# ercembu/bulletproof-perm

Measured on NVIDIA B200. Metric: shuffle proofs/sec prove+verify (52-card), higher is better.
Workload: dtype u32 (8x32-bit limbs, IMAD.WIDE.U32)

## Files before the change

bulletproof-perm_b200/csrc/acproof_kernels.cuh:

```cuda
#pragma once
#include "ge25519.cuh"
#include "vec_kernels.cuh"

struct acp_layout {
    uint32_t n, Q, m, stride;
    uint32_t np, lg;
    uint32_t aL, aR, aO, gamma;
    uint32_t alpha, beta, ro, sl, sr, tau;
    uint32_t y, z, x, w;
    uint32_t yn, yninv, zq;
    uint32_t zWL, zWR, zWO, zWV, zc;
    uint32_t lin, l1, r0, r1, r3;
    uint32_t dots;
    uint32_t tc, tsel, sigma;
    uint32_t l, r, that, taux, mu;
    uint32_t vg, vh, vG, vH, vd;
    uint32_t rho, rho0;
    uint32_t wq, u, uinv, cl, pa, pb, ptab;
    uint32_t stab;
};

#define ACP_PTR(base, lay, p, off) ((base) + 8 * ((size_t)(p) * (lay).stride + (off)))

SC_INLINE uint32_t rotl32(uint32_t v, int n) { return (v << n) | (v >> (32 - n)); }
#define CHACHA_QR(a, b, c, d) \
    a += b; d = rotl32(d ^ a, 16); c += d; b = rotl32(b ^ c, 12); a += b; d = rotl32(d ^ a, 8); c += d; b = rotl32(b ^ c, 7);

__global__ void k_acp_rng(const uint32_t *__restrict__ seeds , acp_layout lay, uint32_t count,
                          uint32_t *__restrict__ blk) {
    const uint32_t j = blockIdx.x * blockDim.x + threadIdx.x, p = blockIdx.y;
    if (j >= count) return;
    uint32_t s[16], x[16];
    s[0] = 0x61707865u; s[1] = 0x3320646eu; s[2] = 0x79622d32u; s[3] = 0x6b206574u;
#pragma unroll
// ... 18 lines not shown
__global__ void __launch_bounds__(128) k_acp_place_witness(const uint32_t *__restrict__ st, acp_layout lay, uint32_t B,
                                                           uint32_t *__restrict__ blk) {
    const uint32_t i = blockIdx.x * blockDim.x + threadIdx.x, p = blockIdx.y;
    const uint32_t n = lay.n, m = lay.m;
    if (i >= 3 * n + m) return;
    const uint32_t which = i < 3 * n ? i / n : 3, k = i - which * n;
    const uint32_t *src = which < 3 ? st + 8 * (((size_t)which * B + p) * n + k) : st + 8 * ((size_t)3 * B * n + (size_t)p * m + k);
    const uint32_t off = which == 0 ? lay.aL : which == 1 ? lay.aR : which == 2 ? lay.aO : lay.gamma;
    uint4 lo = *reinterpret_cast<const uint4 *>(src), hi = *reinterpret_cast<const uint4 *>(src + 4);
    uint32_t *dst = ACP_PTR(blk, lay, p, off + k);
    *reinterpret_cast<uint4 *>(dst) = lo;
    *reinterpret_cast<uint4 *>(dst + 4) = hi;
}

#define WIT_THREADS 256
__global__ void __launch_bounds__(WIT_THREADS) k_shuffle_witness(const uint32_t *__restrict__ deck ,
                                                                 const uint32_t *__restrict__ perm ,
                                                                 const uint32_t *__restrict__ xs , uint32_t k,
                                                                 acp_layout lay, uint32_t *__restrict__ blk,
                                                                 uint32_t *__restrict__ vout ) {
    __shared__ __align__(16) uint32_t sh[2][WIT_THREADS * 8];
    const uint32_t c = blockIdx.x, p = blockIdx.y, tid = threadIdx.x;
    const uint32_t gb = c * (k - 1), vb = c * k, len = k - 1;
    const uint32_t T = blockDim.x;
    const uint32_t run = (len + T - 1) / T, i0 = tid * run, i1 = min(len, i0 + run);
    const uint32_t *pp = perm + (size_t)p * k;
    uint32_t *vp = vout + 8 * (size_t)p * lay.m;
    sc x, one, r2;
    sc_load(x, xs + 8 * (size_t)p);
    sc_const(one, SC_R);
    sc_const(r2, SC_R2);
    auto value = [&](uint32_t j) {
        sc v;
        BPP_ASSERT(j < k && (!c || pp[j] < k));
        sc_load(v, deck + 8 * (size_t)(c ? pp[j] : j));
        sc_store(vp + 8 * (size_t)(vb + j), v);
        return v;
    };
    sc acc = one, f, t;
    for (uint32_t i = i0; i < i1; i++) {
        f = value(i + 1);
        sc_sub(f, f, x);
        sc_store(ACP_PTR(blk, lay, p, lay.aR + gb + i), f);
        sc_mont(t, f, r2);
        sc_mont(acc, acc, t);
    }
    if (tid == 0) {
        f = value(0);
        sc_sub(f, f, x);
        sc_store(ACP_PTR(blk, lay, p, lay.aL + gb), f);
        sc_mont(t, f, r2);
        sc_mont(acc, acc, t);
        if (c == 0) {
            sc_store(vp + 8 * (size_t)(2 * k), x);
            sc z;
            sc_set0(z);
            for (uint32_t q = 2 * k - 2; q < 2 * k; q++) {
                sc_store(ACP_PTR(blk, lay, p, lay.aL + q), z);
                sc_store(ACP_PTR(blk, lay, p, lay.aR + q), z);
                sc_store(ACP_PTR(blk, lay, p, lay.aO + q), z);
            }
        }
    }
    int cur = 0;
    sc_store(sh[0] + 8 * tid, acc);
    __syncthreads();
    for (uint32_t d = 1; d < T; d <<= 1) {
        sc a, b2;
        sc_load(a, sh[cur] + 8 * tid);
// ... 33 lines not shown
    const uint32_t *pp = perm + (size_t)p * k;
    uint32_t *vp = vout + 8 * (size_t)p * lay.m;
    sc x, r2, v, f, fm, P;
    sc_load(x, xs + 8 * (size_t)p);
    sc_const(r2, SC_R2);
    BPP_ASSERT(!c || pp[0] < k);
    sc_load(v, deck + 8 * (size_t)(c ? pp[0] : 0));
    sc_store(vp + 8 * (size_t)vb, v);
    sc_sub(P, v, x);
    sc_store(ACP_PTR(blk, lay, p, lay.aL + gb), P);
#pragma unroll 1
    for (uint32_t i = 0; i < len; i++) {
        BPP_ASSERT(!c || pp[i + 1] < k);
        sc_load(v, deck + 8 * (size_t)(c ? pp[i + 1] : i + 1));
        sc_store(vp + 8 * (size_t)(vb + i + 1), v);
        sc_sub(f, v, x);
        sc_store(ACP_PTR(blk, lay, p, lay.aR + gb + i), f);
        if (i) sc_store(ACP_PTR(blk, lay, p, lay.aL + gb + i), P);
        sc_mont_noinline(fm, f, r2);
        sc_mont_noinline(P, P, fm);
        sc_store(ACP_PTR(blk, lay, p, lay.aO + gb + i), P);
    }
    if (c == 0) {
        sc_store(vp + 8 * (size_t)(2 * k), x);
        sc z;
        sc_set0(z);
        for (uint32_t q = 2 * k - 2; q < 2 * k; q++) {
            sc_store(ACP_PTR(blk, lay, p, lay.aL + q), z);
            sc_store(ACP_PTR(blk, lay, p, lay.aR + q), z);
            sc_store(ACP_PTR(blk, lay, p, lay.aO + q), z);
        }
    }
}
__global__ void __launch_bounds__(128) k_acp_place_gamma(const uint32_t *__restrict__ st, acp_layout lay, uint32_t *__restrict__ blk) {
    const uint32_t i = blockIdx.x * blockDim.x + threadIdx.x, p = blockIdx.y;
    if (i >= lay.m) return;
    const uint32_t *src = st + 8 * ((size_t)p * lay.m + i);
    uint4 lo = *reinterpret_cast<const uint4 *>(src), hi = *reinterpret_cast<const uint4 *>(src + 4);
    uint32_t *dst = ACP_PTR(blk, lay, p, lay.gamma + i);
// ... 40 lines not shown
        ge_affine_to_niels(e, x, y);
        ge_niels_store(dst + FB_ENTRY_U32 * (size_t)(j - 1), e);
        if (j < half) ge_add_noinline(run, run, base);
    }
}

struct fb_shape {
    uint32_t nseg;
    uint32_t sc_off[4];
    uint32_t sc_ostride[4];
    uint32_t gen[4];
    uint32_t cnt[4];
    uint32_t outs;
    uint32_t sel_period;
    uint32_t sel[4];
};
struct fb_consts {
    uint32_t K[8];
};
#ifndef FB_THREADS
#define FB_THREADS 128
#endif
#ifndef FB_GROUP
#define FB_GROUP 4
#endif

static __host__ __device__ __forceinline__ uint32_t fb_terms(const fb_shape &sh) {
    uint32_t n = 0;
    for (uint32_t s = 0; s < sh.nseg; s++) n += sh.cnt[s];
    return n;
// ... 159 lines not shown
            *reinterpret_cast<uint4 *>(stage + 8 * (size_t)t + 4) = hi;
        }
        __syncwarp();
    }
    uint32_t s[9];
    ge_ext acc;
    fb_accumulate_items(acc, s, sh, table, c, Wn, kc, o, total_terms, lane, 32, [&](uint32_t seg, uint32_t k, uint32_t term) {
        return STAGE ? stage + 8 * (size_t)term : fb_scalar(blk, lay, sh, p, o, seg, k);
    });
    ge_warp_sum<false>(acc);
    if (lane == 0) ge_store(out_ext + 32 * ((size_t)p * sh.outs + o), acc);
}
#ifndef FB_STAGE_MAX_BYTES
#define FB_STAGE_MAX_BYTES (48u * 1024u)
#endif
template <int C>
__global__ void __launch_bounds__(FB_THREADS, FB_WARP_MINBLOCKS) k_fb_msm_warp_d(const uint32_t *__restrict__ blk, acp_layout lay, fb_shape sh,
                                                              const uint32_t *__restrict__ table, fb_consts kc,
                                                              uint32_t B, uint32_t outs ,
                                                              uint32_t *__restrict__ out_ext ) {
    constexpr uint32_t WN = (256 + C - 1) / C, LOG_WN = WN == 32 ? 5 : 4, HALF = 1u << (C - 1);
    static_assert((C == 16 && WN == 16) || (C == 8 && WN == 32), "window count must be a power of two dividing 32");
    extern __shared__ __align__(16) uint32_t fb_stage[];
    const uint32_t wid = blockIdx.x * (FB_THREADS / 32) + (threadIdx.x >> 5), lane = threadIdx.x & 31;
    if (wid >= B * outs) return;
    const uint32_t p = wid / outs, o = wid - p * outs;
    const uint32_t total_terms = fb_terms(sh);
    uint32_t *stage = fb_stage + (size_t)(threadIdx.x >> 5) * ((9 * total_terms + 3) & ~3u);
    uint32_t *sgen = stage + 8 * (size_t)total_terms;
    uint32_t n_act = 0;
    for (uint32_t t0 = 0; t0 < total_terms; t0 += 32) {
        const uint32_t t = t0 + lane;
        bool act = t < total_terms;
        uint32_t seg = 0, k = t;
        if (act) {
            fb_locate_term(sh, t, seg, k);
            act = fb_term_selected(sh, seg, k, o);
        }
        const uint32_t bal = __ballot_sync(0xffffffffu, act);
        if (act) {
            const uint32_t idx = n_act + __popc(bal & ((1u << lane) - 1u));
            uint32_t s[8];
            const uint32_t carry = fb_recode(fb_scalar(blk, lay, sh, p, o, seg, k), kc.K, s);
            BPP_ASSERT(carry == 0 && idx < total_terms);
            (void)carry;
            *reinterpret_cast<uint4 *>(stage + 8 * (size_t)idx) = make_uint4(s[0], s[1], s[2], s[3]);
            *reinterpret_cast<uint4 *>(stage + 8 * (size_t)idx + 4) = make_uint4(s[4], s[5], s[6], s[7]);
            sgen[idx] = sh.gen[seg] + k;
        }
        n_act += __popc(bal);
    }
    __syncwarp();
    const uint32_t items = n_act << LOG_WN;
    const uint32_t ww = lane & (WN - 1);
    const bool top = ww == WN - 1;
    const uint32_t lane_entry = ww << (C - 1);
    uint32_t it = lane;
    auto advance = [&](const uint32_t *&ptr, bool &neg) -> bool {
        for (;;) {
            if (it >= items) return false;
            const uint32_t term = it >> LOG_WN;
            it += 32;
            uint32_t u;
            if (C == 16) u = reinterpret_cast<const uint16_t *>(stage)[(term << 4) + ww];
            else u = reinterpret_cast<const uint8_t *>(stage)[(term << 5) + ww];
            const int d = top ? (int)u : (int)u - (int)HALF;
            if (d == 0) continue;
            const uint32_t mag = d < 0 ? (uint32_t)(-d) : (uint32_t)d;
            const uint32_t entry = ((sgen[term] << LOG_WN) << (C - 1)) + lane_entry + (mag - 1);
            BPP_ASSERT(mag >= 1 && mag <= HALF && term < n_act);
            ptr = table + (size_t)entry * FB_ENTRY_U32;
            neg = d < 0;
            return true;
        }
    };
    ge_ext acc;
    fb_accumulate(acc, advance);
    ge_warp_sum<false>(acc);
    if (lane == 0) ge_store(out_ext + 32 * ((size_t)p * sh.outs + o), acc);
}
static inline void fb_warp_launch(const uint32_t *d_sc, const acp_layout &lay, const fb_shape &sh, const uint32_t *table, int c, int Wn,
                                  const fb_consts &kc, uint32_t B, uint32_t outs, uint32_t *d_ext, cudaStream_t st) {
    const uint32_t n_out = B * outs, terms = fb_terms(sh);
    const unsigned grid = (n_out + FB_THREADS / 32 - 1) / (FB_THREADS / 32);
    const size_t stage_d = (size_t)(FB_THREADS / 32) * ((9 * terms + 3) & ~3u) * 4, stage_b = (size_t)(FB_THREADS / 32) * terms * 32;
    uint64_t gen_end = 0;
    for (uint32_t k = 0; k < sh.nseg; k++) gen_end = gen_end > (uint64_t)sh.gen[k] + sh.cnt[k] ? gen_end : (uint64_t)sh.gen[k] + sh.cnt[k];
    const bool fits32 = ((gen_end * Wn) << (c - 1)) < (1ull << 32);
    if (fits32 && stage_d <= FB_STAGE_MAX_BYTES && (c == 16 || c == 8)) {
        if (c == 16) k_fb_msm_warp_d<16><<<grid, FB_THREADS, stage_d, st>>>(d_sc, lay, sh, table, kc, B, outs, d_ext);
        else k_fb_msm_warp_d<8><<<grid, FB_THREADS, stage_d, st>>>(d_sc, lay, sh, table, kc, B, outs, d_ext);
    } else if (stage_b <= FB_STAGE_MAX_BYTES) {
        k_fb_msm_warp<true><<<grid, FB_THREADS, stage_b, st>>>(d_sc, lay, sh, table, c, Wn, kc, B, outs, d_ext);
    } else {
        k_fb_msm_warp<false><<<grid, FB_THREADS, 0, st>>>(d_sc, lay, sh, table, c, Wn, kc, B, outs, d_ext);
    }
}
__global__ void __launch_bounds__(128) k_fb_msm_small(const uint32_t *__restrict__ blk, acp_layout lay, fb_shape sh,
                                                      const uint32_t *__restrict__ table, int c, int Wn, fb_consts kc,
                                                      uint32_t B, uint32_t outs ,
                                                      uint32_t *__restrict__ out_ext ) {
    const uint32_t id = blockIdx.x * blockDim.x + threadIdx.x;
    if (id >= B * outs) return;
    const uint32_t p = id / outs, o = id - p * outs;
    const uint32_t half = 1u << (c - 1);
    ge_ext acc;
// ... 20 lines not shown
}

__global__ void __launch_bounds__(32) k_fb_sum_splits(const uint32_t *__restrict__ part, uint32_t outs, uint32_t splits,
                                                      uint32_t pitch, uint32_t *__restrict__ dst) {
    const uint32_t p = blockIdx.x, o = blockIdx.y, lane = threadIdx.x;
    const uint32_t *src = part + 32 * ((size_t)p * outs + o) * splits;
    ge_ext acc, t;
    ge_identity(acc);
#pragma unroll 1
    for (uint32_t z = lane; z < splits; z += 32) {
        ge_load(t, src + 32 * (size_t)z);
        ge_add(acc, acc, t);
    }
    ge_warp_sum<true>(acc);
    if (lane == 0) ge_store(dst + 32 * ((size_t)p * pitch + o), acc);
}

__global__ void __launch_bounds__(128) k_compress_batch(const uint32_t *__restrict__ ext, uint32_t n,
                                                        uint8_t *__restrict__ out32) {
    uint32_t i = blockIdx.x * blockDim.x + threadIdx.x;
    if (i >= n) return;
    ge_ext p;
    ge_load(p, ext + 32 * (size_t)i);
    ge_compress(out32 + 32 * (size_t)i, p);
}

#define ACP_POW_THREADS 96
__global__ void __launch_bounds__(ACP_POW_THREADS) k_acp_pow(acp_layout lay, uint32_t B, uint32_t *__restrict__ blk) {
    const uint32_t p = blockIdx.x * 32 + (threadIdx.x & 31);
    const int which = threadIdx.x >> 5;
// ... 576 lines not shown
```

bulletproof-perm_b200/csrc/capi_acproof.cu:

```cuda
#include <functional>
#include <thread>

#include "bpperm_internal.hpp"

#include "acproof_kernels.cuh"
#include "ipa_kernels.cuh"
#include "transcript_kernels.cuh"
#include "host_merlin.hpp"


struct bpp_circuit {
    uint32_t n = 0, Q = 0, m = 0, rows = 0, nnz = 0;
    uint32_t *d_rowptr = nullptr, *d_col = nullptr, *d_coeff = nullptr;
    uint8_t *d_kind = nullptr;
    uint32_t n_long = 0, *d_long = nullptr;
};

struct bpp_gens {
    uint32_t n = 0, n_gens = 0;
    bpp_points *pts = nullptr;
};

struct bpp_acp_batch {
    bpp_ctx *ctx = nullptr;
    const bpp_circuit *cir = nullptr;
    const bpp_gens *gens = nullptr;
    int mode = 1;
    uint32_t B = 0, proof_len = 0;
    acp_layout lay;
    std::vector<uint8_t> label;
    uint32_t *d_blk = nullptr, *d_seeds = nullptr, *d_wide = nullptr, *d_ext8 = nullptr, *d_dyn = nullptr,
             *d_wsum = nullptr, *d_stat = nullptr, *d_bad = nullptr, *d_vext = nullptr, *d_vseed = nullptr;
    uint8_t *d_pts8 = nullptr, *d_proofs = nullptr, *d_V = nullptr, *d_accept = nullptr;
    uint8_t *h_pts8 = nullptr, *h_wide = nullptr, *h_proofs = nullptr;
    uint8_t *d_lr = nullptr, *h_lr = nullptr, *h_tx3 = nullptr;
    uint32_t *d_tx3 = nullptr, *d_lrext = nullptr, *d_part = nullptr;
    uint32_t fb_splits = 1;
    bool host_transcripts = false;
    uint64_t *d_tr = nullptr, *d_proto = nullptr;
    uint8_t *d_vdig = nullptr;
    uint32_t *d_wstage = nullptr;
    cudaStream_t aux = nullptr;
    cudaEvent_t ev_fork = nullptr, ev_join = nullptr;
    cudaStream_t aux2 = nullptr;
    cudaEvent_t ev_fork2 = nullptr, ev_join2 = nullptr;
    cudaStream_t aux3 = nullptr;
    cudaEvent_t ev_join3 = nullptr;
    uint32_t *d_vwit = nullptr, *d_wgen = nullptr;
    bool have_vwit = false;
    bool have_V = false;
    uint8_t *h_V = nullptr;
    bool priority_split = false;
    cudaStream_t bulk = nullptr;
    cudaEvent_t ev_bfork = nullptr, ev_bjoin = nullptr;
    bool batch_rlc = true;
    bool decompress_late = false;
    uint32_t *d_rlc_sc = nullptr, *d_rlc_flag = nullptr;
    uint8_t *d_rlc_out = nullptr;
    uint32_t *h_rlc_flag = nullptr;
    std::vector<bpp_host::Transcript> tr;
    bool trace = false;
    std::vector<std::pair<const char *, cudaEvent_t>> marks;
};

// ... 10 lines not shown
static void acp_marks_dump(bpp_acp_batch *b, const char *what) {
    if (!b->trace || b->marks.empty()) return;
    cudaStreamSynchronize(b->ctx->stream);
    fprintf(stderr, "[acp trace] %s:", what);
    for (size_t i = 1; i < b->marks.size(); i++) {
        float ms = 0;
        cudaEventElapsedTime(&ms, b->marks[i - 1].second, b->marks[i].second);
        fprintf(stderr, " %s %.0f us |", b->marks[i].first, ms * 1e3f);
    }
    float tot = 0;
    cudaEventElapsedTime(&tot, b->marks.front().second, b->marks.back().second);
    fprintf(stderr, " total %.0f us\n", tot * 1e3f);
    for (auto &m : b->marks) cudaEventDestroy(m.second);
    b->marks.clear();
}
static acp_layout acp_make_layout(uint32_t n_, uint32_t Q, uint32_t m, int mode) {
    acp_layout L;
    uint32_t o = 0;
    auto take = [&](uint32_t cnt) { uint32_t r = o; o += cnt; return r; };
    L.n = n_; L.Q = Q; L.m = m;
    L.np = mode == 2 ? acp_next_pow2(n_) : n_;
    L.lg = mode == 2 ? acp_log2(L.np) : 0;
    const uint32_t n = L.n, np = L.np;
    L.aL = take(n); L.aR = take(n); L.aO = take(n); L.gamma = take(m);
    L.alpha = take(1); L.beta = take(1); L.ro = take(1); L.sl = take(n); L.sr = take(n); L.tau = take(5);
    L.y = take(1); L.z = take(1); L.x = take(1); L.w = take(1); L.rho0 = take(1);
    L.yn = take(np); L.yninv = take(np); L.zq = take(Q);
    L.zWL = take(n); L.zWR = take(n); L.zWO = take(n); L.zWV = take(m); L.zc = take(1);
    L.lin = take(n); L.l1 = take(n); L.r0 = take(n); L.r1 = take(n); L.r3 = take(n);
    L.dots = take(12); L.sigma = L.dots + 9;
    L.tc = take(6); L.tsel = take(5);
    L.l = take(np); L.r = take(np); L.that = take(1); L.taux = take(1); L.mu = take(1);
    L.vg = take(1); L.vh = take(1); L.vG = take(np); L.vH = take(np); L.vd = take(m + 8 + 2 * L.lg);
    L.wq = take(1); L.u = take(L.lg); L.uinv = take(L.lg); L.cl = take(2); L.pa = take(1); L.pb = take(1);
    L.ptab = take(mode == 2 ? 3 * IPA_MAX_LG : 0);
    L.stab = take(mode == 2 ? 2 * np : 0);
    L.rho = take(1);
    L.stride = (o + 3) & ~3u;
    return L;
}

extern "C" int bpp_circuit_create(bpp_ctx *ctx, size_t n, size_t Q, size_t m, const uint32_t nnz[4], const uint32_t *wire,
                                  const uint32_t *constraint, const uint8_t *coeff, const uint8_t *c_vec,
                                  bpp_circuit **out) {
    if (!ctx || !out || !nnz || n == 0 || Q == 0 || m == 0 || !c_vec) return BPP_ERR_INVALID_ARG;
    *out = nullptr;
    CK(ctx, cudaSetDevice(ctx->device));
    const uint32_t rows = (uint32_t)(3 * n + m + 1);
    const uint32_t row_base[4] = {0, (uint32_t)n, (uint32_t)(2 * n), (uint32_t)(3 * n)};
    const uint32_t row_cnt[4] = {(uint32_t)n, (uint32_t)n, (uint32_t)n, (uint32_t)m};
    size_t total = 0;
    for (int k = 0; k < 4; k++) total += nnz[k];
// ... 116 lines not shown
    int rc = bpp_points_upload(ctx, BPP_FMT_COMPRESSED, all.data(), 2 * n + 2, &pts);
    if (rc) return rc;
    if ((rc = bpp_points_precompute(ctx, pts, window_bits))) {
        bpp_points_free(ctx, pts);
        return rc;
    }
    bpp_gens *gs = new bpp_gens();
    gs->n = (uint32_t)n;
    gs->n_gens = (uint32_t)(2 * n + 2);
    gs->pts = pts;
    *out = gs;
    return BPP_OK;
}
extern "C" void bpp_gens_free(bpp_ctx *ctx, bpp_gens *g) {
    if (!g) return;
    bpp_points_free(ctx, g->pts);
    delete g;
}

__global__ void k_compress_strided(const uint32_t *__restrict__ ext, uint32_t pitch, uint32_t first, uint32_t cnt, uint32_t B,
                                   uint8_t *__restrict__ out32);
extern "C" int bpp_points_precompute(bpp_ctx *ctx, bpp_points *p, int window_bits) {
    if (!ctx || !p || p->n == 0) return BPP_ERR_INVALID_ARG;
    if (window_bits == 0) window_bits = 8;
    if (window_bits < 4 || window_bits > 20) return BPP_ERR_INVALID_ARG;
    CK(ctx, cudaSetDevice(ctx->device));
    if (p->fb_table && p->fb_c == window_bits) return BPP_OK;
    if (p->fb_table) {
        CK(ctx, cudaStreamSynchronize(ctx->stream));
        cudaFree(p->fb_table);
// ... 169 lines not shown
    if (b->h_rlc_flag) cudaFreeHost(b->h_rlc_flag);
    if (b->h_V) cudaFreeHost(b->h_V);
    if (b->aux2) cudaStreamDestroy(b->aux2);
    if (b->aux3) cudaStreamDestroy(b->aux3);
    if (b->ev_join3) cudaEventDestroy(b->ev_join3);
    if (b->ev_fork2) cudaEventDestroy(b->ev_fork2);
    if (b->ev_join2) cudaEventDestroy(b->ev_join2);
    if (b->aux) cudaStreamDestroy(b->aux);
    if (b->bulk) cudaStreamDestroy(b->bulk);
    if (b->ev_bfork) cudaEventDestroy(b->ev_bfork);
    if (b->ev_bjoin) cudaEventDestroy(b->ev_bjoin);
    if (b->ev_fork) cudaEventDestroy(b->ev_fork);
    if (b->ev_join) cudaEventDestroy(b->ev_join);
    delete b;
}

extern "C" int bpp_acp_batch_create(bpp_ctx *ctx, const bpp_circuit *cir, const bpp_gens *gens, int mode, size_t count,
                                    const uint8_t *label, size_t label_len, bpp_acp_batch **out) {
    if (!ctx || !cir || !gens || !out || count == 0 || count > (1u << 24) || mode < 0 || mode > 2 ||
        (!label && label_len))
        return BPP_ERR_INVALID_ARG;
    if (gens->n != (mode == 2 ? acp_next_pow2(cir->n) : cir->n)) return BPP_ERR_LENGTH_MISMATCH;
    if (mode == 2 && acp_log2(acp_next_pow2(cir->n)) > IPA_MAX_LG) return BPP_ERR_INVALID_ARG;
    *out = nullptr;
    CK(ctx, cudaSetDevice(ctx->device));
    bpp_acp_batch *b = new bpp_acp_batch();
    b->ctx = ctx; b->cir = cir; b->gens = gens; b->mode = mode; b->B = (uint32_t)count;
    b->lay = acp_make_layout(cir->n, cir->Q, cir->m, mode);
    b->proof_len = (uint32_t)bpp_acproof_proof_len_mode(cir->n, mode);
    if (const char *e = getenv("BPP_ACP_TRACE")) b->trace = e[0] == '1';
// ... 47 lines not shown
    if (e == cudaSuccess) e = cudaMalloc((void **)&b->d_pts8, B * 8 * 32);
    if (e == cudaSuccess) e = cudaMalloc((void **)&b->d_proofs, B * b->proof_len);
    if (e == cudaSuccess) e = cudaMalloc((void **)&b->d_V, B * cir->m * 32);
    if (e == cudaSuccess) e = cudaMalloc((void **)&b->d_vext, B * cir->m * 128);
    if (e == cudaSuccess) e = cudaMalloc((void **)&b->d_accept, B);
    if (e == cudaSuccess) e = cudaMallocHost((void **)&b->h_pts8, B * 8 * 32);
    if (e == cudaSuccess) e = cudaMallocHost((void **)&b->h_wide, B * nch * 64);
    if (e == cudaSuccess) e = cudaMallocHost((void **)&b->h_proofs, B * b->proof_len);
    if (e != cudaSuccess) {
        ctx->last_error = cudaGetErrorString(e);
        bool oom = e == cudaErrorMemoryAllocation;
        cudaGetLastError();
        bpp_acp_batch_free(b);
        return oom ? BPP_ERR_OOM : BPP_ERR_CUDA;
    }
    *out = b;
    return BPP_OK;
}

extern "C" int bpp_acp_batch_set_priority_split(bpp_acp_batch *b, int on) {
    if (!b) return BPP_ERR_INVALID_ARG;
    bpp_ctx *ctx = b->ctx;
    if (on && !b->bulk) {
        int lo = 0, hi = 0;
        CK(ctx, cudaSetDevice(ctx->device));
        CK(ctx, cudaDeviceGetStreamPriorityRange(&lo, &hi));
        CK(ctx, cudaStreamCreateWithPriority(&b->bulk, cudaStreamNonBlocking, lo));
        CK(ctx, cudaEventCreateWithFlags(&b->ev_bfork, cudaEventDisableTiming));
        CK(ctx, cudaEventCreateWithFlags(&b->ev_bjoin, cudaEventDisableTiming));
    }
// ... 31 lines not shown

static fb_shape acp_shape(uint32_t outs) {
    fb_shape s;
    memset(&s, 0, sizeof(s));
    s.outs = outs;
    return s;
}
static void acp_seg(fb_shape &s, uint32_t off, uint32_t ostride, uint32_t gen, uint32_t cnt) {
    s.sc_off[s.nseg] = off; s.sc_ostride[s.nseg] = ostride; s.gen[s.nseg] = gen; s.cnt[s.nseg] = cnt;
    s.nseg++;
}
static fb_plan acp_fb_plan(const bpp_acp_batch *b, const fb_shape &sh) {
    return fb_choose(b->ctx, (uint64_t)b->B * sh.outs, fb_terms(sh), b->gens->pts->fb_Wn, !sh.sel_period,
                     sh.outs > 8 ? 1 : b->fb_splits);
}
static int fb_launch(bpp_ctx *ctx, const uint32_t *blk, const acp_layout &lay, uint32_t B, const bpp_points &P, const fb_shape &sh,
                     const fb_plan &pl, uint32_t *dst, uint32_t pitch, cudaStream_t st, uint32_t *part, uint32_t *deferred_splits) {
    if (deferred_splits) *deferred_splits = 1;
    fb_shape s = sh;
    s.outs = pitch;
    fb_consts kc;
    memcpy(kc.K, P.fb_K, 32);
    if (pl.form == FB_SMALL) {
        const uint32_t total = B * sh.outs;
        k_fb_msm_small<<<(total + 127) / 128, 128, 0, st>>>(blk, lay, s, P.fb_table, P.fb_c, P.fb_Wn, kc, B, sh.outs, dst);
        LAUNCH_CHECK(ctx);
    } else if (pl.form == FB_WARP) {
        fb_warp_launch(blk, lay, s, P.fb_table, P.fb_c, P.fb_Wn, kc, B, sh.outs, dst, st);
        LAUNCH_CHECK(ctx);
    } else {
        k_fb_msm<<<dim3(B, sh.outs, pl.splits), FB_THREADS, 0, st>>>(blk, lay, s, P.fb_table, P.fb_c, P.fb_Wn, kc,
                                                                    pl.splits > 1 ? part : dst);
        LAUNCH_CHECK(ctx);
        if (pl.splits > 1 && deferred_splits) {
            *deferred_splits = pl.splits;
        } else if (pl.splits > 1) {
            k_fb_sum_splits<<<dim3(B, sh.outs), 32, 0, st>>>(part, sh.outs, pl.splits, pitch, dst);
            LAUNCH_CHECK(ctx);
        }
    }
    return BPP_OK;
}
static int acp_fb(bpp_acp_batch *b, const fb_shape &sh, uint32_t *dst, uint32_t pitch, cudaStream_t on = nullptr,
                  uint32_t part_region = 0, uint32_t *deferred_splits = nullptr) {
    bpp_ctx *ctx = b->ctx;
    const bpp_points &P = *b->gens->pts;
    const fb_plan pl = acp_fb_plan(b, sh);
    uint32_t *part = b->d_part + 32 * (size_t)part_region * b->B * b->fb_splits;
    if (pl.form == FB_SMALL) return fb_launch(ctx, b->d_blk, b->lay, b->B, P, sh, pl, dst, pitch, ctx->stream, part, deferred_splits);
    cudaStream_t st = on ? on : ctx->stream;
    if (b->priority_split && !on) {
        st = b->bulk;
        CK(ctx, cudaEventRecord(b->ev_bfork, ctx->stream));
        CK(ctx, cudaStreamWaitEvent(st, b->ev_bfork, 0));
    }
    int rc = fb_launch(ctx, b->d_blk, b->lay, b->B, P, sh, pl, dst, pitch, st, part, deferred_splits);
    if (rc) return rc;
    if (b->priority_split && !on) {
        CK(ctx, cudaEventRecord(b->ev_bjoin, st));
        CK(ctx, cudaStreamWaitEvent(ctx->stream, b->ev_bjoin, 0));
    }
    return BPP_OK;
}

__global__ void __launch_bounds__(128) k_compress_strided(const uint32_t *__restrict__ ext, uint32_t pitch, uint32_t first,
                                                          uint32_t cnt, uint32_t B, uint8_t *__restrict__ out32) {
    uint32_t id = blockIdx.x * blockDim.x + threadIdx.x;
    if (id >= B * cnt) return;
    uint32_t p = id / cnt, k = first + (id - p * cnt);
    ge_ext pt;
    ge_load(pt, ext + 32 * ((size_t)p * pitch + k));
// ... 6 lines not shown
    bpp_ctx *ctx = b->ctx;
    CK(ctx, cudaSetDevice(ctx->device));
    const size_t n32 = (size_t)b->lay.n * 32 * b->B, m32 = (size_t)b->lay.m * 32 * b->B;
    if (!b->d_wstage) CK(ctx, cudaMalloc((void **)&b->d_wstage, 3 * n32 + m32));
    uint8_t *st = (uint8_t *)b->d_wstage;
    CK(ctx, cudaMemcpyAsync(st, aL, n32, cudaMemcpyHostToDevice, ctx->stream));
    CK(ctx, cudaMemcpyAsync(st + n32, aR, n32, cudaMemcpyHostToDevice, ctx->stream));
    CK(ctx, cudaMemcpyAsync(st + 2 * n32, aO, n32, cudaMemcpyHostToDevice, ctx->stream));
    CK(ctx, cudaMemcpyAsync(st + 3 * n32, gamma, m32, cudaMemcpyHostToDevice, ctx->stream));
    {
        const uint32_t per = 3 * b->lay.n + b->lay.m;
        k_acp_place_witness<<<dim3((per + 127) / 128, b->B), 128, 0, ctx->stream>>>(b->d_wstage, b->lay, b->B, b->d_blk);
        LAUNCH_CHECK(ctx);
    }
    CK(ctx, cudaMemcpyAsync(b->d_seeds, seeds, (size_t)b->B * 32, cudaMemcpyHostToDevice, ctx->stream));
    return BPP_OK;
}

extern "C" int bpp_acp_batch_gen_shuffle_witness(bpp_acp_batch *b, const uint8_t *deck, const uint32_t *perm, const uint8_t *x,
                                                 const uint8_t *gamma, const uint8_t *seeds) {
    if (!b || !deck || !perm || !x || !gamma || !seeds) return BPP_ERR_INVALID_ARG;
    bpp_ctx *ctx = b->ctx;
    CK(ctx, cudaSetDevice(ctx->device));
    const acp_layout &L = b->lay;
    if (L.n < 4 || (L.n & 1u) || L.m != L.n + 1) {
        ctx->last_error = "gen_shuffle_witness: not a shuffle circuit (n = 2k, m = 2k + 1)";
        return BPP_ERR_INVALID_ARG;
    }
    const uint32_t k = L.n / 2, B = b->B;
    const size_t m32 = (size_t)L.m * 32 * B, dk = (size_t)k * 32, pk = (size_t)B * k * 4, xb = (size_t)B * 32;
// ... 6 lines not shown
    CK(ctx, cudaMemcpyAsync(st + m32 + dk + xb, perm, pk, cudaMemcpyHostToDevice, ctx->stream));
    CK(ctx, cudaMemcpyAsync(b->d_seeds, seeds, (size_t)B * 32, cudaMemcpyHostToDevice, ctx->stream));
    k_acp_place_gamma<<<dim3((L.m + 127) / 128, B), 128, 0, ctx->stream>>>((const uint32_t *)st, L, b->d_blk);
    LAUNCH_CHECK(ctx);
    if (k <= 64 || (k <= 1024 && 2ull * B >= 2048)) {
        k_shuffle_witness_serial<<<(2 * B + 63) / 64, 64, 0, ctx->stream>>>((const uint32_t *)(st + m32), (const uint32_t *)(st + m32 + dk + xb),
                                                                           (const uint32_t *)(st + m32 + dk), k, B, L, b->d_blk, b->d_vwit);
    } else {
        unsigned wit_threads = 32;
        while (wit_threads < WIT_THREADS && wit_threads < k - 1) wit_threads <<= 1;
        k_shuffle_witness<<<dim3(2, B), wit_threads, 0, ctx->stream>>>((const uint32_t *)(st + m32), (const uint32_t *)(st + m32 + dk + xb),
                                                                      (const uint32_t *)(st + m32 + dk), k, L, b->d_blk, b->d_vwit);
    }
    LAUNCH_CHECK(ctx);
    b->have_vwit = true;
    return BPP_OK;
}

extern "C" int bpp_acp_batch_commit(bpp_acp_batch *b, const uint8_t *v, uint8_t *V_out) {
    if (!b || (!v && !b->have_vwit)) return BPP_ERR_INVALID_ARG;
    bpp_ctx *ctx = b->ctx;
    CK(ctx, cudaSetDevice(ctx->device));
    const acp_layout &L = b->lay;
    if (2 * L.n < L.m) return BPP_ERR_INVALID_ARG;
    const size_t pitch = (size_t)L.stride * 32, m32 = (size_t)L.m * 32;
    CK(ctx, cudaMemcpy2DAsync((uint8_t *)b->d_blk + 32 * (size_t)L.l, pitch, v ? (const void *)v : (const void *)b->d_vwit, m32, m32, b->B,
                              v ? cudaMemcpyHostToDevice : cudaMemcpyDeviceToDevice, ctx->stream));
    fb_shape sh = acp_shape(L.m);
    acp_seg(sh, L.l, 1, 0, 1);
    acp_seg(sh, L.gamma, 1, 1, 1);
// ... 233 lines not shown
        ctx->last_error = "prove: the value commitments are not resident (bpp_acp_batch_commit / _upload_commitments)";
        return BPP_ERR_INVALID_ARG;
    }
    if (bind_V && !b->host_transcripts && (rc = acp_fork_vchunks(b))) return rc;
    acp_mark(b, "start");
    const uint32_t nrand = 3 + 2 * n + 5;
    k_acp_rng<<<dim3((nrand + 127) / 128, B), 128, 0, s>>>(b->d_seeds, L, nrand, b->d_blk);
    LAUNCH_CHECK(ctx);
    {
        const bool side = b->fb_splits > 1 && !b->priority_split && b->aux3;
        if (side) {
            CK(ctx, cudaEventRecord(b->ev_fork, s));
            CK(ctx, cudaStreamWaitEvent(b->aux, b->ev_fork, 0));
            CK(ctx, cudaStreamWaitEvent(b->aux3, b->ev_fork, 0));
        }
        fb_shape sh = acp_shape(1);
        const uint32_t gH = 2 + b->gens->n;
        acp_seg(sh, L.alpha, 0, 1, 1); acp_seg(sh, L.aL, 0, 2, n); acp_seg(sh, L.aR, 0, gH, n);
        if ((rc = acp_fb(b, sh, b->d_ext8 + 0, 8))) return rc;
        sh = acp_shape(1);
        acp_seg(sh, L.beta, 0, 1, 1); acp_seg(sh, L.aO, 0, 2, n);
        if ((rc = acp_fb(b, sh, b->d_ext8 + 32, 8, side ? b->aux : nullptr, side ? 1 : 0))) return rc;
        sh = acp_shape(1);
        acp_seg(sh, L.ro, 0, 1, 1); acp_seg(sh, L.sl, 0, 2, n); acp_seg(sh, L.sr, 0, gH, n);
        if ((rc = acp_fb(b, sh, b->d_ext8 + 64, 8, side ? b->aux3 : nullptr, side ? 2 : 0))) return rc;
        if (side) {
            CK(ctx, cudaEventRecord(b->ev_join, b->aux));
            CK(ctx, cudaEventRecord(b->ev_join3, b->aux3));
            CK(ctx, cudaStreamWaitEvent(s, b->ev_join, 0));
            CK(ctx, cudaStreamWaitEvent(s, b->ev_join3, 0));
        }
    }
    acp_mark(b, "rng+A_I,A_O,S");
    k_compress_strided<<<(B * 3 + 127) / 128, 128, 0, s>>>(b->d_ext8, 8, 0, 3, B, b->d_pts8);
// ... 332 lines not shown

extern "C" int bpp_acp_batch_download_accept(bpp_acp_batch *b, uint8_t *accept) {
    if (!b || !accept) return BPP_ERR_INVALID_ARG;
    bpp_ctx *ctx = b->ctx;
    CK(ctx, cudaMemcpyAsync(accept, b->d_accept, b->B, cudaMemcpyDeviceToHost, ctx->stream));
    CK(ctx, cudaStreamSynchronize(ctx->stream));
    return BPP_OK;
}

extern "C" int bpp_acp_batch_time_commit_msm(bpp_acp_batch *b, int reps, float *ms_avg, uint64_t *mixed_adds,
                                             uint64_t *full_adds) {
    if (!b || reps <= 0 || !ms_avg) return BPP_ERR_INVALID_ARG;
    bpp_ctx *ctx = b->ctx;
    CK(ctx, cudaSetDevice(ctx->device));
    const acp_layout &L = b->lay;
    fb_shape sh = acp_shape(1);
    acp_seg(sh, L.alpha, 0, 1, 1); acp_seg(sh, L.aL, 0, 2, L.n); acp_seg(sh, L.aR, 0, 2 + b->gens->n, L.n);
    int rc = acp_fb(b, sh, b->d_ext8, 8);
    if (rc) return rc;
    cudaEvent_t e0, e1;
    cudaEventCreate(&e0);
    cudaEventCreate(&e1);
    cudaEventRecord(e0, ctx->stream);
    for (int i = 0; i < reps; i++)
        if ((rc = acp_fb(b, sh, b->d_ext8, 8))) return rc;
    cudaEventRecord(e1, ctx->stream);
    CK(ctx, cudaEventSynchronize(e1));
    float ms = 0;
    cudaEventElapsedTime(&ms, e0, e1);
    cudaEventDestroy(e0);
    cudaEventDestroy(e1);
    *ms_avg = ms / reps;
// ... 381 lines not shown
```

Before: 693,400.

## Exploit shuffle witness structure in A_I commitment via H-sum and sparse digit lists

For shuffle-shaped circuits, the A_I commitment MSM over aR = v - x is rewritten as an MSM over the raw card values v plus a single term -x against a precomputed sum of the H generators. That sum is computed once per generator set and cached with its own fixed-base table. Because card values are small, their recoded digits are mostly neutral, so the warp kernel gains a sparse path: terms with at most two nonzero digits go into a compact per-warp list instead of the full digit scan. This cuts table lookups and point additions in the commitment, at the cost of a new kernel template, extra shared memory, a one-time setup launch, and more complex eligibility checks.

```diff
diff --git a/bulletproof-perm_b200/csrc/acproof_kernels.cuh b/bulletproof-perm_b200/csrc/acproof_kernels.cuh
--- a/bulletproof-perm_b200/csrc/acproof_kernels.cuh
+++ b/bulletproof-perm_b200/csrc/acproof_kernels.cuh
@@ -18,6 +18,7 @@
     uint32_t rho, rho0;
     uint32_t wq, u, uinv, cl, pa, pb, ptab;
     uint32_t stab;
+    uint32_t vr, nx;
 };
 
 #define ACP_PTR(base, lay, p, off) ((base) + 8 * ((size_t)(p) * (lay).stride + (off)))
@@ -66,6 +67,12 @@
 }
 
 #define WIT_THREADS 256
+SC_INLINE void acp_store_neg_x(uint32_t *blk, const acp_layout &lay, uint32_t p, const sc &x) {
+    sc z, nx;
+    sc_set0(z);
+    sc_sub(nx, z, x);
+    sc_store(ACP_PTR(blk, lay, p, lay.nx), nx);
+}
 __global__ void __launch_bounds__(WIT_THREADS) k_shuffle_witness(const uint32_t *__restrict__ deck ,
                                                                  const uint32_t *__restrict__ perm ,
                                                                  const uint32_t *__restrict__ xs , uint32_t k,
@@ -92,6 +99,7 @@
     sc acc = one, f, t;
     for (uint32_t i = i0; i < i1; i++) {
         f = value(i + 1);
+        sc_store(ACP_PTR(blk, lay, p, lay.vr + gb + i), f);
         sc_sub(f, f, x);
         sc_store(ACP_PTR(blk, lay, p, lay.aR + gb + i), f);
         sc_mont(t, f, r2);
@@ -105,6 +113,7 @@
         sc_mont(acc, acc, t);
         if (c == 0) {
             sc_store(vp + 8 * (size_t)(2 * k), x);
+            acp_store_neg_x(blk, lay, p, x);
             sc z;
             sc_set0(z);
             for (uint32_t q = 2 * k - 2; q < 2 * k; q++) {
@@ -168,6 +177,7 @@
         BPP_ASSERT(!c || pp[i + 1] < k);
         sc_load(v, deck + 8 * (size_t)(c ? pp[i + 1] : i + 1));
         sc_store(vp + 8 * (size_t)(vb + i + 1), v);
+        sc_store(ACP_PTR(blk, lay, p, lay.vr + gb + i), v);
         sc_sub(f, v, x);
         sc_store(ACP_PTR(blk, lay, p, lay.aR + gb + i), f);
         if (i) sc_store(ACP_PTR(blk, lay, p, lay.aL + gb + i), P);
@@ -177,6 +187,7 @@
     }
     if (c == 0) {
         sc_store(vp + 8 * (size_t)(2 * k), x);
+        acp_store_neg_x(blk, lay, p, x);
         sc z;
         sc_set0(z);
         for (uint32_t q = 2 * k - 2; q < 2 * k; q++) {
@@ -247,6 +258,10 @@
     uint32_t outs;
     uint32_t sel_period;
     uint32_t sel[4];
+};
+struct fb_sparse {
+    uint32_t on, alt;
+    const uint32_t *alt_table;
 };
 struct fb_consts {
     uint32_t K[8];
@@ -436,9 +451,18 @@
 #ifndef FB_STAGE_MAX_BYTES
 #define FB_STAGE_MAX_BYTES (48u * 1024u)
 #endif
+#define FB_SPARSE_MAX 2
+#define FB_ALT 0x80000000u
+static __host__ __device__ __forceinline__ uint32_t fb_stage_d_words(uint32_t terms, bool sparse) {
+    return ((9 * terms + 3) & ~3u) + (sparse ? FB_SPARSE_MAX * terms : 0);
+}
 template <int C>
+__device__ __forceinline__ uint32_t fb_field(const uint32_t (&s)[8], uint32_t w) {
+    return C == 16 ? (s[w >> 1] >> (16 * (w & 1))) & 0xffffu : (s[w >> 2] >> (8 * (w & 3))) & 0xffu;
+}
+template <int C, bool SPARSE>
 __global__ void __launch_bounds__(FB_THREADS, FB_WARP_MINBLOCKS) k_fb_msm_warp_d(const uint32_t *__restrict__ blk, acp_layout lay, fb_shape sh,
-                                                              const uint32_t *__restrict__ table, fb_consts kc,
+                                                              const uint32_t *__restrict__ table, fb_consts kc, fb_sparse sp,
                                                               uint32_t B, uint32_t outs ,
                                                               uint32_t *__restrict__ out_ext ) {
     constexpr uint32_t WN = (256 + C - 1) / C, LOG_WN = WN == 32 ? 5 : 4, HALF = 1u << (C - 1);
@@ -448,27 +472,59 @@
     if (wid >= B * outs) return;
     const uint32_t p = wid / outs, o = wid - p * outs;
     const uint32_t total_terms = fb_terms(sh);
-    uint32_t *stage = fb_stage + (size_t)(threadIdx.x >> 5) * ((9 * total_terms + 3) & ~3u);
+    const uint32_t lt = (1u << lane) - 1u;
+    uint32_t *stage = fb_stage + (size_t)(threadIdx.x >> 5) * fb_stage_d_words(total_terms, SPARSE);
     uint32_t *sgen = stage + 8 * (size_t)total_terms;
-    uint32_t n_act = 0;
+    uint32_t *slist = stage + fb_stage_d_words(total_terms, false);
+    uint32_t n_act = 0, n_sp = 0;
     for (uint32_t t0 = 0; t0 < total_terms; t0 += 32) {
         const uint32_t t = t0 + lane;
         bool act = t < total_terms;
-        uint32_t seg = 0, k = t;
+        uint32_t seg = 0, k = t, gen = 0;
+        uint32_t s[8];
         if (act) {
             fb_locate_term(sh, t, seg, k);
             act = fb_term_selected(sh, seg, k, o);
         }
+        if (act) {
+            const uint32_t carry = fb_recode(fb_scalar(blk, lay, sh, p, o, seg, k), kc.K, s);
+            BPP_ASSERT(carry == 0);
+            (void)carry;
+            gen = sh.gen[seg] + k;
+            if (SPARSE && ((sp.alt >> seg) & 1u)) gen |= FB_ALT;
+        }
+        if (SPARSE) {
+            uint32_t nz = 0;
+            if (act && !(gen & FB_ALT)) {
+#pragma unroll
+                for (uint32_t w = 0; w < WN; w++) nz += fb_field<C>(s, w) != (w == WN - 1 ? 0u : HALF);
+            }
+            const bool sp = act && !(gen & FB_ALT) && nz <= FB_SPARSE_MAX;
+            static_assert(FB_SPARSE_MAX == 2, "the list positions below count terms of one and of two digits");
+            const uint32_t b1 = __ballot_sync(0xffffffffu, sp && nz == 1), b2 = __ballot_sync(0xffffffffu, sp && nz == 2);
+            if (sp) {
+                uint32_t pos = n_sp + __popc(b1 & lt) + 2 * __popc(b2 & lt);
+#pragma unroll
+                for (uint32_t w = 0; w < WN; w++) {
+                    const uint32_t u = fb_field<C>(s, w);
+                    const int d = w == WN - 1 ? (int)u : (int)u - (int)HALF;
+                    if (d != 0) {
+                        const uint32_t mag = d < 0 ? (uint32_t)(-d) : (uint32_t)d;
+                        BPP_ASSERT(pos < FB_SPARSE_MAX * total_terms);
+                        slist[pos++] = ((((gen << LOG_WN) + w) << (C - 1)) + (mag - 1)) << 1 | (d < 0 ? 1u : 0u);
+                    }
+                }
+            }
+            n_sp += __popc(b1) + 2 * __popc(b2);
+            act = act && !sp;
+        }
         const uint32_t bal = __ballot_sync(0xffffffffu, act);
         if (act) {
-            const uint32_t idx = n_act + __popc(bal & ((1u << lane) - 1u));
-            uint32_t s[8];
-            const uint32_t carry = fb_recode(fb_scalar(blk, lay, sh, p, o, seg, k), kc.K, s);
-            BPP_ASSERT(carry == 0 && idx < total_terms);
-            (void)carry;
+            const uint32_t idx = n_act + __popc(bal & lt);
+            BPP_ASSERT(idx < total_terms);
             *reinterpret_cast<uint4 *>(stage + 8 * (size_t)idx) = make_uint4(s[0], s[1], s[2], s[3]);
             *reinterpret_cast<uint4 *>(stage + 8 * (size_t)idx + 4) = make_uint4(s[4], s[5], s[6], s[7]);
-            sgen[idx] = sh.gen[seg] + k;
+            sgen[idx] = gen;
         }
         n_act += __popc(bal);
     }
@@ -478,9 +534,17 @@
     const bool top = ww == WN - 1;
     const uint32_t lane_entry = ww << (C - 1);
     uint32_t it = lane;
+    uint32_t js = (lane - items) & 31u;
     auto advance = [&](const uint32_t *&ptr, bool &neg) -> bool {
         for (;;) {
-            if (it >= items) return false;
+            if (it >= items) {
+                if (!SPARSE || js >= n_sp) return false;
+                const uint32_t wd = slist[js];
+                js += 32;
+                ptr = table + (size_t)(wd >> 1) * FB_ENTRY_U32;
+                neg = wd & 1u;
+                return true;
+            }
             const uint32_t term = it >> LOG_WN;
             it += 32;
             uint32_t u;
@@ -489,9 +553,10 @@
             const int d = top ? (int)u : (int)u - (int)HALF;
             if (d == 0) continue;
             const uint32_t mag = d < 0 ? (uint32_t)(-d) : (uint32_t)d;
-            const uint32_t entry = ((sgen[term] << LOG_WN) << (C - 1)) + lane_entry + (mag - 1);
+            const uint32_t g = sgen[term];
+            const uint32_t entry = ((g << LOG_WN) << (C - 1)) + lane_entry + (mag - 1);
             BPP_ASSERT(mag >= 1 && mag <= HALF && term < n_act);
-            ptr = table + (size_t)entry * FB_ENTRY_U32;
+            ptr = (SPARSE && (g & FB_ALT) ? sp.alt_table : table) + (size_t)entry * FB_ENTRY_U32;
             neg = d < 0;
             return true;
         }
@@ -501,17 +566,28 @@
     ge_warp_sum<false>(acc);
     if (lane == 0) ge_store(out_ext + 32 * ((size_t)p * sh.outs + o), acc);
 }
+static inline bool fb_warp_d_fits(const fb_shape &sh, const fb_sparse &sp, int c, int Wn) {
+    uint64_t gen_end = 0;
+    for (uint32_t k = 0; k < sh.nseg; k++) {
+        const uint64_t e = ((sp.alt >> k) & 1u) ? 1 : (uint64_t)sh.gen[k] + sh.cnt[k];
+        gen_end = gen_end > e ? gen_end : e;
+    }
+    const bool fits = ((gen_end * Wn) << (c - 1)) < (sp.on ? 1ull << 31 : 1ull << 32);
+    const size_t stage_d = (size_t)(FB_THREADS / 32) * fb_stage_d_words(fb_terms(sh), sp.on != 0) * 4;
+    return fits && stage_d <= FB_STAGE_MAX_BYTES && (c == 16 || c == 8);
+}
 static inline void fb_warp_launch(const uint32_t *d_sc, const acp_layout &lay, const fb_shape &sh, const uint32_t *table, int c, int Wn,
-                                  const fb_consts &kc, uint32_t B, uint32_t outs, uint32_t *d_ext, cudaStream_t st) {
+                                  const fb_consts &kc, uint32_t B, uint32_t outs, uint32_t *d_ext, cudaStream_t st,
+                                  const fb_sparse &sp = fb_sparse{}) {
     const uint32_t n_out = B * outs, terms = fb_terms(sh);
     const unsigned grid = (n_out + FB_THREADS / 32 - 1) / (FB_THREADS / 32);
-    const size_t stage_d = (size_t)(FB_THREADS / 32) * ((9 * terms + 3) & ~3u) * 4, stage_b = (size_t)(FB_THREADS / 32) * terms * 32;
-    uint64_t gen_end = 0;
-    for (uint32_t k = 0; k < sh.nseg; k++) gen_end = gen_end > (uint64_t)sh.gen[k] + sh.cnt[k] ? gen_end : (uint64_t)sh.gen[k] + sh.cnt[k];
-    const bool fits32 = ((gen_end * Wn) << (c - 1)) < (1ull << 32);
-    if (fits32 && stage_d <= FB_STAGE_MAX_BYTES && (c == 16 || c == 8)) {
-        if (c == 16) k_fb_msm_warp_d<16><<<grid, FB_THREADS, stage_d, st>>>(d_sc, lay, sh, table, kc, B, outs, d_ext);
-        else k_fb_msm_warp_d<8><<<grid, FB_THREADS, stage_d, st>>>(d_sc, lay, sh, table, kc, B, outs, d_ext);
+    const size_t stage_d = (size_t)(FB_THREADS / 32) * fb_stage_d_words(terms, sp.on != 0) * 4,
+                 stage_b = (size_t)(FB_THREADS / 32) * terms * 32;
+    if (fb_warp_d_fits(sh, sp, c, Wn)) {
+        if (sp.on && c == 16) k_fb_msm_warp_d<16, true><<<grid, FB_THREADS, stage_d, st>>>(d_sc, lay, sh, table, kc, sp, B, outs, d_ext);
+        else if (sp.on) k_fb_msm_warp_d<8, true><<<grid, FB_THREADS, stage_d, st>>>(d_sc, lay, sh, table, kc, sp, B, outs, d_ext);
+        else if (c == 16) k_fb_msm_warp_d<16, false><<<grid, FB_THREADS, stage_d, st>>>(d_sc, lay, sh, table, kc, sp, B, outs, d_ext);
+        else k_fb_msm_warp_d<8, false><<<grid, FB_THREADS, stage_d, st>>>(d_sc, lay, sh, table, kc, sp, B, outs, d_ext);
     } else if (stage_b <= FB_STAGE_MAX_BYTES) {
         k_fb_msm_warp<true><<<grid, FB_THREADS, stage_b, st>>>(d_sc, lay, sh, table, c, Wn, kc, B, outs, d_ext);
     } else {
@@ -562,6 +638,20 @@
     }
     ge_warp_sum<true>(acc);
     if (lane == 0) ge_store(dst + 32 * ((size_t)p * pitch + o), acc);
+}
+
+__global__ void __launch_bounds__(32) k_point_sum(const uint32_t *__restrict__ niels, uint32_t first, uint32_t cnt,
+                                                  uint32_t *__restrict__ out_ext) {
+    ge_ext acc;
+    ge_identity(acc);
+#pragma unroll 1
+    for (uint32_t i = threadIdx.x; i < cnt; i += 32) {
+        ge_niels q;
+        ge_niels_load(q, niels + 24 * (size_t)(first + i));
+        ge_madd(acc, acc, q, false);
+    }
+    ge_warp_sum<true>(acc);
+    if (threadIdx.x == 0) ge_store(out_ext, acc);
 }
 
 __global__ void __launch_bounds__(128) k_compress_batch(const uint32_t *__restrict__ ext, uint32_t n,
diff --git a/bulletproof-perm_b200/csrc/capi_acproof.cu b/bulletproof-perm_b200/csrc/capi_acproof.cu
--- a/bulletproof-perm_b200/csrc/capi_acproof.cu
+++ b/bulletproof-perm_b200/csrc/capi_acproof.cu
@@ -19,6 +19,9 @@
 struct bpp_gens {
     uint32_t n = 0, n_gens = 0;
     bpp_points *pts = nullptr;
+    struct range_sum { uint32_t first, cnt; bpp_points *pts; };
+    std::vector<range_sum> sums;
+    std::mutex mu;
 };
 
 struct bpp_acp_batch {
@@ -48,6 +51,8 @@
     cudaEvent_t ev_join3 = nullptr;
     uint32_t *d_vwit = nullptr, *d_wgen = nullptr;
     bool have_vwit = false;
+    bool shuffle_wit = false;
+    const bpp_points *hsum = nullptr;
     bool have_V = false;
     uint8_t *h_V = nullptr;
     bool priority_split = false;
@@ -88,6 +93,7 @@
     for (auto &m : b->marks) cudaEventDestroy(m.second);
     b->marks.clear();
 }
+static bool acp_shuffle_shaped(uint32_t n, uint32_t m) { return n >= 4 && !(n & 1u) && m == n + 1; }
 static acp_layout acp_make_layout(uint32_t n_, uint32_t Q, uint32_t m, int mode) {
     acp_layout L;
     uint32_t o = 0;
@@ -110,6 +116,8 @@
     L.ptab = take(mode == 2 ? 3 * IPA_MAX_LG : 0);
     L.stab = take(mode == 2 ? 2 * np : 0);
     L.rho = take(1);
+    const bool shuffle = acp_shuffle_shaped(n, m);
+    L.vr = take(shuffle ? n - 2 : 0); L.nx = take(shuffle ? 1 : 0);
     L.stride = (o + 3) & ~3u;
     return L;
 }
@@ -256,6 +264,7 @@
 }
 extern "C" void bpp_gens_free(bpp_ctx *ctx, bpp_gens *g) {
     if (!g) return;
+    for (auto &e : g->sums) bpp_points_free(ctx, e.pts);
     bpp_points_free(ctx, g->pts);
     delete g;
 }
@@ -455,6 +464,8 @@
     if (b->ev_join) cudaEventDestroy(b->ev_join);
     delete b;
 }
+
+static int acp_prepare_hsum(bpp_acp_batch *b);
 
 extern "C" int bpp_acp_batch_create(bpp_ctx *ctx, const bpp_circuit *cir, const bpp_gens *gens, int mode, size_t count,
                                     const uint8_t *label, size_t label_len, bpp_acp_batch **out) {
@@ -532,6 +543,10 @@
         bpp_acp_batch_free(b);
         return oom ? BPP_ERR_OOM : BPP_ERR_CUDA;
     }
+    if (int rc = acp_prepare_hsum(b)) {
+        bpp_acp_batch_free(b);
+        return rc;
+    }
     *out = b;
     return BPP_OK;
 }
@@ -593,9 +608,75 @@
     return fb_choose(b->ctx, (uint64_t)b->B * sh.outs, fb_terms(sh), b->gens->pts->fb_Wn, !sh.sel_period,
                      sh.outs > 8 ? 1 : b->fb_splits);
 }
+static fb_shape acp_ai_shape(const bpp_acp_batch *b, bool structured, fb_sparse *sp = nullptr) {
+    const acp_layout &L = b->lay;
+    const uint32_t gH = 2 + b->gens->n;
+    fb_shape sh = acp_shape(1);
+    acp_seg(sh, L.alpha, 0, 1, 1); acp_seg(sh, L.aL, 0, 2, L.n);
+    if (!structured) {
+        acp_seg(sh, L.aR, 0, gH, L.n);
+        return sh;
+    }
+    acp_seg(sh, L.vr, 0, gH, L.n - 2); acp_seg(sh, L.nx, 0, 0, 1);
+    if (sp) *sp = fb_sparse{1, 1u << 3, b->hsum ? b->hsum->fb_table : nullptr};
+    return sh;
+}
+static bool acp_ai_structured_ok(const bpp_acp_batch *b) {
+    if (!acp_shuffle_shaped(b->lay.n, b->lay.m)) return false;
+    const bpp_points &P = *b->gens->pts;
+    fb_sparse sp;
+    const fb_shape sh = acp_ai_shape(b, true, &sp);
+    return acp_fb_plan(b, sh).form == FB_WARP && fb_warp_d_fits(sh, sp, P.fb_c, P.fb_Wn);
+}
+static int acp_prepare_hsum(bpp_acp_batch *b) {
+    if (!acp_ai_structured_ok(b)) return BPP_OK;
+    bpp_ctx *ctx = b->ctx;
+    bpp_gens *g = const_cast<bpp_gens *>(b->gens);
+    const uint32_t first = 2 + g->n, cnt = b->lay.n - 2;
+    const int c = g->pts->fb_c;
+    std::lock_guard<std::mutex> lock(g->mu);
+    for (const auto &e : g->sums)
+        if (e.first == first && e.cnt == cnt && e.pts->fb_c == c) {
+            b->hsum = e.pts;
+            return BPP_OK;
+        }
+    uint32_t *d = nullptr;
+    CK(ctx, cudaMalloc((void **)&d, 128 + 32));
+    uint8_t enc[32];
+    k_point_sum<<<1, 32, 0, ctx->stream>>>(g->pts->niels, first, cnt, d);
+    cudaError_t e = cudaGetLastError();
+    if (e == cudaSuccess) {
+        k_compress_batch<<<1, 128, 0, ctx->stream>>>(d, 1, (uint8_t *)(d + 32));
+        e = cudaGetLastError();
+    }
+    if (e == cudaSuccess) e = cudaMemcpyAsync(enc, d + 32, 32, cudaMemcpyDeviceToHost, ctx->stream);
+    if (e == cudaSuccess) e = cudaStreamSynchronize(ctx->stream);
+    cudaFree(d);
+    if (e != cudaSuccess) {
+        ctx->last_error = cudaGetErrorString(e);
+        return BPP_ERR_CUDA;
+    }
+    ctx->launches += 2;
+    bpp_points *pts = nullptr;
+    int rc = bpp_points_upload(ctx, BPP_FMT_COMPRESSED, enc, 1, &pts);
+    if (rc) return rc;
+    if ((rc = bpp_points_precompute(ctx, pts, c))) {
+        bpp_points_free(ctx, pts);
+        return rc;
+    }
+    g->sums.push_back({first, cnt, pts});
+    b->hsum = pts;
+    return BPP_OK;
+}
+
 static int fb_launch(bpp_ctx *ctx, const uint32_t *blk, const acp_layout &lay, uint32_t B, const bpp_points &P, const fb_shape &sh,
-                     const fb_plan &pl, uint32_t *dst, uint32_t pitch, cudaStream_t st, uint32_t *part, uint32_t *deferred_splits) {
+                     const fb_plan &pl, uint32_t *dst, uint32_t pitch, cudaStream_t st, uint32_t *part, uint32_t *deferred_splits,
+                     const fb_sparse &sp = fb_sparse{}) {
     if (deferred_splits) *deferred_splits = 1;
+    if ((sp.on || sp.alt) && !(pl.form == FB_WARP && fb_warp_d_fits(sh, sp, P.fb_c, P.fb_Wn))) {
+        ctx->last_error = "fixed-base MSM: a sparse / two-table shape needs the digit-staged warp form";
+        return BPP_ERR_INVALID_ARG;
+    }
     fb_shape s = sh;
     s.outs = pitch;
     fb_consts kc;
@@ -605,7 +686,7 @@
         k_fb_msm_small<<<(total + 127) / 128, 128, 0, st>>>(blk, lay, s, P.fb_table, P.fb_c, P.fb_Wn, kc, B, sh.outs, dst);
         LAUNCH_CHECK(ctx);
     } else if (pl.form == FB_WARP) {
-        fb_warp_launch(blk, lay, s, P.fb_table, P.fb_c, P.fb_Wn, kc, B, sh.outs, dst, st);
+        fb_warp_launch(blk, lay, s, P.fb_table, P.fb_c, P.fb_Wn, kc, B, sh.outs, dst, st, sp);
         LAUNCH_CHECK(ctx);
     } else {
         k_fb_msm<<<dim3(B, sh.outs, pl.splits), FB_THREADS, 0, st>>>(blk, lay, s, P.fb_table, P.fb_c, P.fb_Wn, kc,
@@ -621,19 +702,19 @@
     return BPP_OK;
 }
 static int acp_fb(bpp_acp_batch *b, const fb_shape &sh, uint32_t *dst, uint32_t pitch, cudaStream_t on = nullptr,
-                  uint32_t part_region = 0, uint32_t *deferred_splits = nullptr) {
+                  uint32_t part_region = 0, uint32_t *deferred_splits = nullptr, const fb_sparse &sp = fb_sparse{}) {
     bpp_ctx *ctx = b->ctx;
     const bpp_points &P = *b->gens->pts;
     const fb_plan pl = acp_fb_plan(b, sh);
     uint32_t *part = b->d_part + 32 * (size_t)part_region * b->B * b->fb_splits;
-    if (pl.form == FB_SMALL) return fb_launch(ctx, b->d_blk, b->lay, b->B, P, sh, pl, dst, pitch, ctx->stream, part, deferred_splits);
+    if (pl.form == FB_SMALL) return fb_launch(ctx, b->d_blk, b->lay, b->B, P, sh, pl, dst, pitch, ctx->stream, part, deferred_splits, sp);
     cudaStream_t st = on ? on : ctx->stream;
     if (b->priority_split && !on) {
         st = b->bulk;
         CK(ctx, cudaEventRecord(b->ev_bfork, ctx->stream));
         CK(ctx, cudaStreamWaitEvent(st, b->ev_bfork, 0));
     }
-    int rc = fb_launch(ctx, b->d_blk, b->lay, b->B, P, sh, pl, dst, pitch, st, part, deferred_splits);
+    int rc = fb_launch(ctx, b->d_blk, b->lay, b->B, P, sh, pl, dst, pitch, st, part, deferred_splits, sp);
     if (rc) return rc;
     if (b->priority_split && !on) {
         CK(ctx, cudaEventRecord(b->ev_bjoin, st));
@@ -670,6 +751,7 @@
         LAUNCH_CHECK(ctx);
     }
     CK(ctx, cudaMemcpyAsync(b->d_seeds, seeds, (size_t)b->B * 32, cudaMemcpyHostToDevice, ctx->stream));
+    b->shuffle_wit = false;
     return BPP_OK;
 }
 
@@ -706,6 +788,7 @@
     }
     LAUNCH_CHECK(ctx);
     b->have_vwit = true;
+    b->shuffle_wit = true;
     return BPP_OK;
 }
 
@@ -969,10 +1052,12 @@
             CK(ctx, cudaStreamWaitEvent(b->aux, b->ev_fork, 0));
             CK(ctx, cudaStreamWaitEvent(b->aux3, b->ev_fork, 0));
         }
-        fb_shape sh = acp_shape(1);
+        const bpp_points &P = *b->gens->pts;
+        const bool structured = b->shuffle_wit && b->hsum && b->hsum->fb_c == P.fb_c && acp_ai_structured_ok(b);
+        fb_sparse sp{};
+        fb_shape sh = acp_ai_shape(b, structured, &sp);
+        if ((rc = acp_fb(b, sh, b->d_ext8 + 0, 8, nullptr, 0, nullptr, sp))) return rc;
         const uint32_t gH = 2 + b->gens->n;
-        acp_seg(sh, L.alpha, 0, 1, 1); acp_seg(sh, L.aL, 0, 2, n); acp_seg(sh, L.aR, 0, gH, n);
-        if ((rc = acp_fb(b, sh, b->d_ext8 + 0, 8))) return rc;
         sh = acp_shape(1);
         acp_seg(sh, L.beta, 0, 1, 1); acp_seg(sh, L.aO, 0, 2, n);
         if ((rc = acp_fb(b, sh, b->d_ext8 + 32, 8, side ? b->aux : nullptr, side ? 1 : 0))) return rc;
@@ -1335,8 +1420,7 @@
     bpp_ctx *ctx = b->ctx;
     CK(ctx, cudaSetDevice(ctx->device));
     const acp_layout &L = b->lay;
-    fb_shape sh = acp_shape(1);
-    acp_seg(sh, L.alpha, 0, 1, 1); acp_seg(sh, L.aL, 0, 2, L.n); acp_seg(sh, L.aR, 0, 2 + b->gens->n, L.n);
+    const fb_shape sh = acp_ai_shape(b, false);
     int rc = acp_fb(b, sh, b->d_ext8, 8);
     if (rc) return rc;
     cudaEvent_t e0, e1;
```

New measurement: 741,500 (median of 6 runs). 1.07x the previous value.
